# tsadja/ShaSTA

Measured on AMD Instinct MI355X. Metric: affinity frame-pairs/sec at N=M=500, F=256, higher is better.
Workload: dtype f32; 1 GPU; synthetic N=M=500, F=256 (num_point 4 x C 64), nf=7: affinity forward from HBM-resident NHWC BEV maps (SURVEY 8a rows 4-16); max_obj=500, num_feats=7, num_point=4, arithmetic=f16x2, parallelism=replica x1

## Files before the change

### shasta_amd/csrc/pair.hip

```cpp
#include "stages.hpp"
#include "pair_lane.hpp"

namespace shasta {

struct PackArgs {
    shasta_linear fs[4], fd[3], rc[3], aff0;
    float* out;
    int N, nf, F;
};

__device__ __forceinline__ void layer_src(const PackArgs& a, int l, const float*& W, const float*& b, int& ldw) {
    const PairDims d(a.F);
    switch (l) {
        case L_FS2: W = a.fs[1].weight; b = a.fs[1].bias; ldw = d.H1; break;
        case L_FS3: W = a.fs[2].weight; b = a.fs[2].bias; ldw = d.H2; break;
        case L_FS4: W = a.fs[3].weight; b = a.fs[3].bias; ldw = d.H3; break;
        case L_RC2: W = a.rc[1].weight; b = a.rc[1].bias; ldw = d.R1; break;
        case L_RC3: W = a.rc[2].weight; b = a.rc[2].bias; ldw = d.R2; break;
        case L_FD2: W = a.fd[1].weight; b = a.fd[1].bias; ldw = 32; break;
        default:    W = a.fd[2].weight; b = a.fd[2].bias; ldw = 8; break;
    }
}

__global__ void pack_pair_weights_kernel(PackArgs a) {
// ... 289 lines not shown
#pragma unroll
        for (int i = 0; i < TPI; ++i) dma_up(t + 2 * TPI + i, (t - t_beg + 2 * TPI + i) % RING);
        const int tt = t + th;
        unsigned upo = (unsigned)(unsigned long long)(my_up + ((t - t_beg + th) % RING) * UP_SLOT);
        asm volatile("" : "+v"(upo));
        const lfloat* up = (const lfloat*)(unsigned long long)upo;
        float hp[16];
        {
            const f32x4 h0 = *reinterpret_cast<const lf32x4*>(up + ET), h1 = *reinterpret_cast<const lf32x4*>(up + ET + 4),
                        h2 = *reinterpret_cast<const lf32x4*>(up + ET + 8), h3 = *reinterpret_cast<const lf32x4*>(up + ET + 12);
#pragma unroll
            for (int k = 0; k < 4; ++k) {
                hp[k] = h0[k];
                hp[4 + k] = h1[k];
                hp[8 + k] = h2[k];
                hp[12 + k] = h3[k];
            }
        }
        const lfloat *arow, *abias;
        a4l.per_track(arow, abias);

        auto layer12 = [&](auto tag, int seg, f32x4* acc) {
            using AL = decltype(tag);
            a4_init<AL>(abias, acc);
#pragma unroll
            for (int kg = 0; kg < AL::KG; ++kg) {
                const f32x4 u = *reinterpret_cast<const f32x4*>(ucrow + seg + 4 * kg);
                const f32x4 upv = *reinterpret_cast<const lf32x4*>(up + seg + 4 * kg);
                f32x4 a4[AL::NOB];
#pragma unroll
                for (int ob = 0; ob < AL::NOB; ++ob) a4[ob] = *reinterpret_cast<const lf32x4*>(arow + AL::OFF + (ob * AL::KG + kg) * 16);
#pragma unroll
                for (int kk = 0; kk < 4; ++kk) {
                    if (4 * kg + kk < AL::KIN) {
                        const float h = relu_nan(upv[kk] + u[kk]);
#pragma unroll
                        for (int ob = 0; ob < AL::NOB; ++ob) acc[ob] = MFMA4(a4[ob][kk], h, acc[ob]);
                    }
                }
            }
        };
        f32x4 a_rc2[A4<F, L_RC2>::NOB], a_rc3[A4<F, L_RC3>::NOB];
        f32x4 a_fs2[A4<F, L_FS2>::NOB], a_fs3[A4<F, L_FS3>::NOB], a_fs4[A4<F, L_FS4>::NOB];
        f32x4 a_fd2[A4<F, L_FD2>::NOB], a_fd3[A4<F, L_FD3>::NOB];
        layer12(A4<F, L_RC2>{}, H1, a_rc2);
        layer12(A4<F, L_FS2>{}, 0, a_fs2);
        layer12(A4<F, L_FD2>{}, H1 + R1, a_fd2);
        a4_layer<A4<F, L_RC3>, A4_RELU_NAN>(arow, abias, a_rc2, a_rc3);
        a4_layer<A4<F, L_FS3>, A4_RELU_NAN>(arow, abias, a_fs2, a_fs3);
        a4_layer<A4<F, L_FD3>, A4_RELU_NAN>(arow, abias, a_fd2, a_fd3);
        a4_layer<A4<F, L_FS4>, A4_RELU_NAN>(arow, abias, a_fs3, a_fs4);

        const float dist = hand_dist(hp, hd, dnm, rdn);
        const float res = pair_combine(a_rc3[0], a_fd3[0][0], dist, a_fs4[0][0]);
        if (d < D && tt < t_end) residual[((size_t)b * T + tt) * ld + d] = res;
    }
}

int pair_residual(const shasta_weights* w, const float* packed, int B, const float* feat, const float* prev_feat,
                  const float* det_tab, const float* prev_tab, float* residual, int ld, void* ws, size_t ws_bytes,
                  hipStream_t st, hipEvent_t ev0, hipEvent_t ev1) {
    const int N = w->max_obj, F = w->feat_dim, nf = w->num_feats, T = N + 2, D = N + 2;
    const PairDims d(F);
    const PackedLayout P(N, nf, F);
    const PairWs L(B, N, F);
    if (ws_bytes < L.total) {
        set_error_msg("pair_residual: workspace too small");
        return SHASTA_E_WORKSPACE;
    }
    if (B == 0) return SHASTA_OK;
    char* base = static_cast<char*>(ws);
    float* UP = reinterpret_cast<float*>(base + L.up);
    float* UC = reinterpret_cast<float*>(base + L.uc);
    float* hand_prev = reinterpret_cast<float*>(base + L.hand_prev);
// ... 112 lines not shown
```

### shasta_amd/csrc/pair_f16.hip

```cpp
#include "stages.hpp"
#include "pair_lane.hpp"
#include "pieces.hpp"

namespace shasta {


constexpr int P16_FRAG_DW = 2 * 4 * 64 * 4;

__global__ __launch_bounds__(256) void pair_f16_pack_kernel(PairF16PackArgs a) {
    __shared__ float red[3][4];
    __shared__ int ex[3];
    const int tid = threadIdx.x;
    const float* W[3] = {a.w_fs2, a.w_rc2, a.w_fd2};
    const int cnt[3] = {16 * 32, 16 * 64, 8 * 32};
    pair2_range_exponents(W, cnt, a.out, P16_FRAG_DW, red, ex);
    const int lane = tid & 63, frag = tid >> 6;
    const int i = lane & 15, kb = lane >> 4;
    const int mlp = frag == 0 ? 0 : frag == 3 ? 2 : 1;
    const int rows = mlp == 2 ? 8 : 16, kin = mlp == 1 ? 64 : 32, ks = frag == 2 ? 1 : 0;
    float v[8];
#pragma unroll
    for (int j = 0; j < 8; ++j) v[j] = i < rows ? __builtin_ldexpf(W[mlp][i * kin + 32 * ks + 8 * kb + j], ex[mlp]) : 0.0f;
    store_weight_pieces(v, a.out, 4, frag, lane);
}

int pair_f16_pack(const shasta_weights* w, float* out, hipStream_t st) {
    hipLaunchKernelGGL(pair_f16_pack_kernel, dim3(1), dim3(256), 0, st, pair_f16_pack_args(w, out));
    return check_launch("pair_f16_pack");
}

constexpr int PF_TS = 44;
constexpr int GR_ROW = 136;

template <int WPB, bool GRID>
struct PairF16Lds {
    static constexpr int US = PairDims(256).ET + 4;
    static constexpr int uc = 0;
    static constexpr int ucl = uc + 64 * (GR_ROW / 2);
    static constexpr int a4 = uc + (GRID ? 2 * 64 * (GR_ROW / 2) : 64 * US);
    static constexpr int up = a4 + pad4(a4_total(256));
    static constexpr int tr = up + WPB * 3 * UP_SLOT;
    static constexpr int upp = tr + WPB * 64 * PF_TS;
    static constexpr size_t bytes = (size_t)(upp + (GRID ? WPB * 128 : 0)) * sizeof(float);
};
static_assert(PairF16Lds<8, false>::bytes == 156912 && PairF16Lds<8, true>::bytes == 162032, "the sizes the launcher spelt out before");


template <int WPB, bool GRID>
__global__ __launch_bounds__(64 * WPB) void pair_f16_kernel(const float* __restrict__ packed, const uint32_t* __restrict__ p16,
                                                       const float* __restrict__ UP, const float* __restrict__ UC,
                                                       const float* __restrict__ hand_prev, const float* __restrict__ hand_det,
                                                       const float* __restrict__ denom, float* __restrict__ residual, int T,
                                                       int D, int ld, int nf, int TWG, int TA, int TB) {
    constexpr int F = 256;
    constexpr PairDims dm(F);
    constexpr int ET = dm.ET;
    static_assert(dm.H1 == 32 && dm.R1 == 64 && ET == 128 && dm.H2 == 16 && dm.R2 == 16, "pair_f16_kernel is laid out for F = 256");
    using Lds = PairF16Lds<WPB, GRID>;
    constexpr int US = Lds::US;
    extern __shared__ __attribute__((aligned(16))) float s_dynh[];
    float* s_uc = s_dynh + Lds::uc;
    float* s_a4 = s_dynh + Lds::a4;
    float* s_up = s_dynh + Lds::up;
    float* s_tr = s_dynh + Lds::tr;
    uint32_t* s_uch = reinterpret_cast<uint32_t*>(s_dynh + Lds::uc);
    uint32_t* s_ucl = reinterpret_cast<uint32_t*>(s_dynh + Lds::ucl);
    uint32_t* s_upp = reinterpret_cast<uint32_t*>(s_dynh + Lds::upp);
    const int tid = threadIdx.x, lane = tid & 63;
    const int wid = __builtin_amdgcn_readfirstlane(tid >> 6);
    int lbx, by, b;
    xcd_logical_block(lbx, by, b);
    const int d0 = lbx * 64;
    const int d = d0 + lane, dcl = min(d, D - 1);
    {
        if constexpr (!GRID) {
            const f32x4* src = reinterpret_cast<const f32x4*>(UC);
#pragma unroll 4
            for (int e = tid; e < 64 * (ET / 4); e += 64 * WPB) {
                const int r = e / (ET / 4), c = e - r * (ET / 4);
                const int cp = (((c >> 1) & 1) << 4) | (((c >> 2) & 1) << 3) | ((c >> 3) << 1) | (c & 1);
                *reinterpret_cast<f32x4*>(&s_uc[r * US + 4 * cp]) = src[((size_t)b * D + min(d0 + r, D - 1)) * (ET / 4) + c];
            }
        }
        a4_stage<F, 64 * WPB>(packed, s_a4, tid);
    }
    float hd[12];
    float mc = load_hand_det(hand_det + ((size_t)b * D + dcl) * 16, hd);
// ... 48 lines not shown
            _Float16 hh[4], ll[4];
#pragma unroll
            for (int q = 0; q < 4; ++q) {
                const float sv = __builtin_ldexpf(v[q], ex), hi = rintf(sv);
                hh[q] = (_Float16)hi;
                ll[q] = (_Float16)(rintf((sv - hi) * 2048.0f) * (1.0f / 2048.0f));
            }
            typedef uint32_t pu2 __attribute__((ext_vector_type(2)));
            typedef _Float16 ph2t __attribute__((ext_vector_type(2)));
            *reinterpret_cast<pu2*>(s_uch + r * (GR_ROW / 2) + 2 * c) =
                pu2{__builtin_bit_cast(uint32_t, ph2t{hh[0], hh[1]}), __builtin_bit_cast(uint32_t, ph2t{hh[2], hh[3]})};
            *reinterpret_cast<pu2*>(s_ucl + r * (GR_ROW / 2) + 2 * c) =
                pu2{__builtin_bit_cast(uint32_t, ph2t{ll[0], ll[1]}), __builtin_bit_cast(uint32_t, ph2t{ll[2], ll[3]})};
        }
    }
    u32x4 wh[4], wl[4];
#pragma unroll
    for (int f = 0; f < 4; ++f) {
        wh[f] = reinterpret_cast<const u32x4*>(p16)[(0 * 4 + f) * 64 + lane];
        wl[f] = reinterpret_cast<const u32x4*>(p16)[(1 * 4 + f) * 64 + lane];
    }
    const int ew_fs = reinterpret_cast<const int*>(p16)[P16_FRAG_DW + 0], ew_rc = reinterpret_cast<const int*>(p16)[P16_FRAG_DW + 1],
              ew_fd = reinterpret_cast<const int*>(p16)[P16_FRAG_DW + 2];
    __syncthreads();
    const A4Lane a4l(s_a4, lane);
    const f32x4 zero4 = {0, 0, 0, 0};
    const int p = lane & 15, kb = lane >> 4;
    float* my_tr = s_tr + wid * (64 * PF_TS);

    const int t_beg = by * TWG + (wid < 4 ? wid * TA : 4 * TA + (wid - 4) * TB);
    const int t_end = min(min(T, (by + 1) * TWG), t_beg + (wid < 4 ? TA : TB));
    float* my_up = s_up + wid * (3 * UP_SLOT);
    const bool hp_lane = lane >= ET / 4 && lane < ET / 4 + 4;
    const int up_lane = 4 * min(lane, ET / 4 - 1), hp_off = 4 * (lane - ET / 4);
    auto dma_up = [&](int row, int slot) {
        const size_t r = (size_t)b * T + min(row, T - 1);
        const float* src = hp_lane ? hand_prev + r * 16 + hp_off : UP + r * ET + up_lane;
        __builtin_amdgcn_global_load_lds((const __attribute__((address_space(1))) void*)src,
                                         (__attribute__((address_space(3))) void*)(my_up + slot * UP_SLOT), 16, 0, 0);
    };
    if (t_beg < t_end) {
        dma_up(t_beg, 0);
        dma_up(t_beg + 1, 1);
    }
    for (int t = t_beg; t < t_end; ++t) {
        asm volatile("s_waitcnt vmcnt(0)" ::: "memory");
        dma_up(t + 2, (t - t_beg + 2) % 3);
        unsigned upo = (unsigned)(unsigned long long)(my_up + ((t - t_beg) % 3) * UP_SLOT);
// ... 124 lines not shown
        {
            f32x4 ua[8], ub[8];
            u32x4 xha[4], xla[4], xhb[4], xlb[4];
            f32x4 fsA, rcA, fdA, fsB, rcB, fdB;
            load_uc(0, ua);
            load_uc(1, ub);
            cut(ua, xha, xla);
            load_uc(2, ua);
            cut(ub, xhb, xlb);
            mma(xha, xla, fsA, rcA, fdA);
            store(0, fsA, rcA, fdA);
            load_uc(3, ub);
            cut(ua, xha, xla);
            mma(xhb, xlb, fsB, rcB, fdB);
            store(1, fsB, rcB, fdB);
            cut(ub, xhb, xlb);
            mma(xha, xla, fsA, rcA, fdA);
            store(2, fsA, rcA, fdA);
            mma(xhb, xlb, fsB, rcB, fdB);
            store(3, fsB, rcB, fdB);
        }
        const lfloat *arow, *abias;
        a4l.per_track(arow, abias);
        const float i_rc = __builtin_ldexpf(1.0f, -((GRID ? ge[1] : e1) + ew_rc)), i_fs = __builtin_ldexpf(1.0f, -((GRID ? ge[0] : e1) + ew_fs)),
                    i_fd = __builtin_ldexpf(1.0f, -((GRID ? ge[2] : e1) + ew_fd));
        f32x4 a_rc2[4], a_fs2[4], a_fd2[2];
        {
            const float* mine = my_tr + lane * PF_TS;
            const float* b_rc = s_a4 + A4<F, L_RC2>::OFF + A4<F, L_RC2>::BIAS;
            const float* b_fs = s_a4 + A4<F, L_FS2>::OFF + A4<F, L_FS2>::BIAS;
            const float* b_fd = s_a4 + A4<F, L_FD2>::OFF + A4<F, L_FD2>::BIAS;
#pragma unroll
            for (int g = 0; g < 4; ++g) {
                a_rc2[g] = a4_descale_relu(*reinterpret_cast<const f32x4*>(mine + 4 * g), i_rc, *reinterpret_cast<const f32x4*>(b_rc + 4 * g));
                a_fs2[g] = a4_descale_relu(*reinterpret_cast<const f32x4*>(mine + 16 + 4 * g), i_fs, *reinterpret_cast<const f32x4*>(b_fs + 4 * g));
            }
#pragma unroll
            for (int g = 0; g < 2; ++g)
                a_fd2[g] = a4_descale_relu(*reinterpret_cast<const f32x4*>(mine + 32 + 4 * g), i_fd, *reinterpret_cast<const f32x4*>(b_fd + 4 * g));
        }
        asm volatile("" : "+v"(a_rc2[0]), "+v"(a_rc2[1]), "+v"(a_rc2[2]), "+v"(a_rc2[3]), "+v"(a_fs2[0]), "+v"(a_fs2[1]), "+v"(a_fs2[2]),
                     "+v"(a_fs2[3]), "+v"(a_fd2[0]), "+v"(a_fd2[1]));
        f32x4 a_rc3[A4<F, L_RC3>::NOB], a_fs3[A4<F, L_FS3>::NOB], a_fs4[A4<F, L_FS4>::NOB], a_fd3[A4<F, L_FD3>::NOB];
        {
            using RC = A4<F, L_RC3>;
            using FS = A4<F, L_FS3>;
            using FD = A4<F, L_FD3>;
            static_assert(RC::NOB == 1 && FS::NOB == 2 && FD::NOB == 1 && RC::KG == 4 && FS::KG == 4 && FD::KG == 2, "F = 256");
            a4_init<RC>(abias, a_rc3);
            a4_init<FS>(abias, a_fs3);
            a4_init<FD>(abias, a_fd3);
#pragma unroll
            for (int kg = 0; kg < 4; ++kg) {
                const f32x4 w_rc = *reinterpret_cast<const lf32x4*>(arow + RC::OFF + kg * 16);
                const f32x4 w_f0 = *reinterpret_cast<const lf32x4*>(arow + FS::OFF + kg * 16);
                const f32x4 w_f1 = *reinterpret_cast<const lf32x4*>(arow + FS::OFF + (FS::KG + kg) * 16);
                f32x4 w_fd = zero4;
                if (kg < 2) w_fd = *reinterpret_cast<const lf32x4*>(arow + FD::OFF + kg * 16);
#pragma unroll
                for (int kk = 0; kk < 4; ++kk) {
                    a_rc3[0] = MFMA4(w_rc[kk], a_rc2[kg][kk], a_rc3[0]);
                    a_fs3[0] = MFMA4(w_f0[kk], a_fs2[kg][kk], a_fs3[0]);
                    a_fs3[1] = MFMA4(w_f1[kk], a_fs2[kg][kk], a_fs3[1]);
                    if (kg < 2) a_fd3[0] = MFMA4(w_fd[kk], a_fd2[kg][kk], a_fd3[0]);
                }
            }
        }
        a4_layer<A4<F, L_FS4>, A4_RELU_FMAX>(arow, abias, a_fs3, a_fs4);

        const float dist = hand_dist(hp, hd, dnm, rdn);
        const float res = pair_combine(a_rc3[0], a_fd3[0][0], dist, a_fs4[0][0]);
        if (d < D) residual[((size_t)b * T + t) * ld + d] = finite_bound ? res : __builtin_nanf("");
    }
}

int launch_pair_f16(const float* packed, const float* p16, const float* UP, const float* UC, const float* hand_prev,
                    const float* hand_det, const float* denom, float* residual, int B, int T, int D, int ld, int nf, bool grid,
                    hipStream_t st) {
    constexpr int wpb = 8;
    int ny = 1;
    while ((long)B * cdiv(D, 64) * ny < 512 && cdiv(T, wpb * ny * 2) >= 2) ny *= 2;
    const int twg = cdiv(cdiv(T, ny), wpb) * wpb;
    int ta = twg / wpb, tb = ta;
    if (wpb == 8) {
        const int per_simd = twg / 4;
        ta = (per_simd * 1000 + (1000 + 615) / 2) / (1000 + 615);
        tb = per_simd - ta;
    }
    const size_t lds = grid ? PairF16Lds<wpb, true>::bytes : PairF16Lds<wpb, false>::bytes;
    dim3 grd(cdiv(D, 64), cdiv(T, twg), B);
    if (grid) {
        (void)hipFuncSetAttribute((const void*)pair_f16_kernel<wpb, true>, hipFuncAttributeMaxDynamicSharedMemorySize, (int)lds);
        hipLaunchKernelGGL((pair_f16_kernel<wpb, true>), grd, dim3(64 * wpb), lds, st, packed, reinterpret_cast<const uint32_t*>(p16), UP, UC,
                           hand_prev, hand_det, denom, residual, T, D, ld, nf, twg, ta, tb);
    } else {
// ... 9 lines not shown
```

### shasta_amd/csrc/pair_f16w.hip

```cpp
#include "stages.hpp"
#include "pair_lane.hpp"
#include "pieces.hpp"

namespace shasta {

template <int F>
struct PW {
    static constexpr PairDims dm{F};
    static constexpr int ET = dm.ET, H1 = dm.H1, R1 = dm.R1, H2 = dm.H2, R2 = dm.R2, NKS = ET / 16;
    static_assert(ET % 16 == 0 && H2 % 4 == 0 && H2 + 8 <= 32 && R2 <= 32, "wide pair tiles: 16-wide k steps, two 32-row output blocks");
    static constexpr bool has1(int ks) { return 16 * ks < H1 || 16 * ks + 16 > H1 + R1; }
    static constexpr bool has2(int ks) { return 16 * ks + 16 > H1 && 16 * ks < H1 + R1; }
    static constexpr int frag1(int ks) {
        int f = 0;
        for (int i = 0; i < ks; ++i) f += (has1(i) ? 1 : 0) + (has2(i) ? 1 : 0);
        return f;
    }
    static constexpr int frag2(int ks) { return frag1(ks) + (has1(ks) ? 1 : 0); }
    static constexpr int NFRAG = frag1(NKS);
    static constexpr int FRAG_DW = 2 * NFRAG * 64 * 4;
};
constexpr int P16W_MAX_DW = 2 * 16 * 64 * 4 + 4;
static_assert(PW<320>::FRAG_DW + 4 <= P16W_MAX_DW && PW<256>::FRAG_DW + 4 <= P16W_MAX_DW, "PackedLayout::p16w");

__device__ __forceinline__ f32x2 w_mul2(f32x2 a, f32x2 c) {
    f32x2 r;
    asm("v_pk_mul_f32 %0, %1, %2" : "=v"(r) : "v"(a), "v"(c));
    return r;
}

struct PairF16WPackArgs : PairF16PackArgs {};

template <int F>
__global__ __launch_bounds__(256) void pair_f16w_pack_kernel(PairF16WPackArgs a) {
    using W = PW<F>;
    __shared__ float red[3][4];
    __shared__ int ex[3];
    const int tid = threadIdx.x;
    const float* Wm[3] = {a.w_fs2, a.w_rc2, a.w_fd2};
    const int cnt[3] = {W::H2 * W::H1, W::R2 * W::R1, 8 * 32};
    pair2_range_exponents(Wm, cnt, a.out, W::FRAG_DW, red, ex);
    const int lane = tid & 63, m = lane & 31, kb = lane >> 5;
    for (int item = tid >> 6; item < 2 * W::NKS; item += 4) {
        const int ks = item >> 1, blk = item & 1;
        if (!(blk == 0 ? W::has1(ks) : W::has2(ks))) continue;
        const int frag = blk == 0 ? W::frag1(ks) : W::frag2(ks);
        float v[8];
#pragma unroll
        for (int j = 0; j < 8; ++j) {
            const int c = 16 * ks + 8 * kb + j;
            float x = 0.0f;
            if (blk == 0) {
                if (m < W::H2 && c < W::H1) x = __builtin_ldexpf(a.w_fs2[m * W::H1 + c], ex[0]);
                else if (m >= W::H2 && m < W::H2 + 8 && c >= W::H1 + W::R1) x = __builtin_ldexpf(a.w_fd2[(m - W::H2) * 32 + (c - W::H1 - W::R1)], ex[2]);
            } else if (m < W::R2 && c >= W::H1 && c < W::H1 + W::R1) {
                x = __builtin_ldexpf(a.w_rc2[m * W::R1 + (c - W::H1)], ex[1]);
            }
            v[j] = x;
        }
        store_weight_pieces(v, a.out, W::NFRAG, frag, lane);
    }
}

bool pair_f16w_serves(int F) { return F == 320; }

int pair_f16w_pack(const shasta_weights* w, float* out, hipStream_t st) {
    hipLaunchKernelGGL(pair_f16w_pack_kernel<320>, dim3(1), dim3(256), 0, st, PairF16WPackArgs{pair_f16_pack_args(w, out)});
    return check_launch("pair_f16w_pack");
}

constexpr int PWK_WPB = 4;

template <int F>
struct PairF16wLds {
    static constexpr int a4 = 0;
    static constexpr int up = a4 + pad4(a4_total(F));
    static constexpr int w = up + PWK_WPB * 6 * UP_SLOT;
    static constexpr size_t bytes = (size_t)(w + PW<F>::FRAG_DW) * sizeof(float);
};
static_assert(PairF16wLds<320>::bytes == 56928, "the size the launcher spelt out before");

template <int F>
__global__ __launch_bounds__(64 * PWK_WPB) __attribute__((amdgpu_waves_per_eu(2, 2))) void pair_f16w_kernel(const float* __restrict__ packed, const uint32_t* __restrict__ p16,
                                                               const float* __restrict__ UP, const float* __restrict__ UC,
                                                               const float* __restrict__ hand_prev, const float* __restrict__ hand_det,
                                                               const float* __restrict__ denom, float* __restrict__ residual, int T,
                                                               int D, int ld, int TWG) {
    using W = PW<F>;
    constexpr int ET = W::ET, NKS = W::NKS, NFRAG = W::NFRAG;
    using Lds = PairF16wLds<F>;
    extern __shared__ __attribute__((aligned(16))) float s_dynw[];
    float* s_a4 = s_dynw + Lds::a4;
    float* s_up = s_dynw + Lds::up;
    u32x4* s_w = reinterpret_cast<u32x4*>(s_dynw + Lds::w);
    const int tid = threadIdx.x, lane = tid & 63;
    const int wid = __builtin_amdgcn_readfirstlane(tid >> 6);
    int lbx, by, b;
    xcd_logical_block(lbx, by, b);
    const int d0 = lbx * 32;
    const int n = lane & 31, kb = lane >> 5;
    const int d = d0 + n, dcl = min(d, D - 1);
    a4_stage<F, 64 * PWK_WPB>(packed, s_a4, tid);
    f32x4 uc[NKS][2];
    {
        const f32x4* src = reinterpret_cast<const f32x4*>(UC + ((size_t)b * D + dcl) * ET);
#pragma unroll
        for (int ks = 0; ks < NKS; ++ks) {
            uc[ks][0] = src[4 * ks + 2 * kb];
            uc[ks][1] = src[4 * ks + 2 * kb + 1];
        }
    }
    float hd[12];
    float mc = load_hand_det(hand_det + ((size_t)b * D + dcl) * 16, hd);
#pragma unroll
    for (int off = 16; off > 0; off >>= 1) mc = absmax_keep_nan(mc, __shfl_xor(mc, off, 64));
    const float dnm = denom[(size_t)b * D + dcl], rdn = 1.0f / dnm;
    for (int e = tid; e < 2 * NFRAG * 64; e += 64 * PWK_WPB) s_w[e] = reinterpret_cast<const u32x4*>(p16)[e];
    const u32x4* my_w = s_w + lane;
    const int ew_fs = reinterpret_cast<const int*>(p16)[W::FRAG_DW + 0], ew_rc = reinterpret_cast<const int*>(p16)[W::FRAG_DW + 1],
              ew_fd = reinterpret_cast<const int*>(p16)[W::FRAG_DW + 2];
    __syncthreads();
    const A4Lane a4l(s_a4, lane);
    const f32x4 zero4 = {0, 0, 0, 0};
    const f32x16 zero16 = {0, 0, 0, 0, 0, 0, 0, 0, 0, 0, 0, 0, 0, 0, 0, 0};

    const int tw = TWG / PWK_WPB;
    const int t_beg = by * TWG + wid * tw;
    const int t_end = min(min(T, (by + 1) * TWG), t_beg + tw);
    float* my_up = s_up + wid * (6 * UP_SLOT);
    const bool hp_lane = lane >= ET / 4 && lane < ET / 4 + 4;
    const int up_lane = 4 * min(lane, ET / 4 - 1), hp_off = 4 * (lane - ET / 4);
    auto dma_up = [&](int row, int slot) __attribute__((always_inline)) {
        const size_t r = (size_t)b * T + min(row, T - 1);
        const float* src = hp_lane ? hand_prev + r * 16 + hp_off : UP + r * ET + up_lane;
        __builtin_amdgcn_global_load_lds((const __attribute__((address_space(1))) void*)src,
                                         (__attribute__((address_space(3))) void*)(my_up + slot * UP_SLOT), 16, 0, 0);
    };
    if (t_beg < t_end) {
        dma_up(t_beg, 0);
        dma_up(t_beg + 1, 1);
        dma_up(t_beg + 2, 2);
        dma_up(t_beg + 3, 3);
    }
// ... 95 lines not shown
                    q2[2 * g][r] = __uint_as_float(s2[0]);
                    q2[2 * g + 1][r] = __uint_as_float(s2[1]);
                }
            }
        const int my_t = t + kb;
        const lfloat* upL = upA + kb * UP_SLOT;
        float hp[16];
        {
            const f32x4 h0 = *reinterpret_cast<const lf32x4*>(upL + ET), h1 = *reinterpret_cast<const lf32x4*>(upL + ET + 4),
                        h2 = *reinterpret_cast<const lf32x4*>(upL + ET + 8), h3 = *reinterpret_cast<const lf32x4*>(upL + ET + 12);
#pragma unroll
            for (int k = 0; k < 4; ++k) {
                hp[k] = h0[k];
                hp[4 + k] = h1[k];
                hp[8 + k] = h2[k];
                hp[12 + k] = h3[k];
            }
        }
        const float bound = kb ? boundB : boundA;
        const bool finite_bound = bound < INFINITY;
        const int e1 = kb ? e1B : e1A;
        const lfloat *arow, *abias;
        a4l.per_track(arow, abias);
        const float i_rc = __builtin_ldexpf(1.0f, -(e1 + ew_rc)), i_fs = __builtin_ldexpf(1.0f, -(e1 + ew_fs)), i_fd = __builtin_ldexpf(1.0f, -(e1 + ew_fd));
        constexpr int NQ_FS = W::H2 / 4, NQ_RC = (W::R2 + 3) / 4;
        f32x4 a_fs2[NQ_FS], a_rc2[NQ_RC], a_fd2[2];
        {
            const float* b_rc = s_a4 + A4<F, L_RC2>::OFF + A4<F, L_RC2>::BIAS;
            const float* b_fs = s_a4 + A4<F, L_FS2>::OFF + A4<F, L_FS2>::BIAS;
            const float* b_fd = s_a4 + A4<F, L_FD2>::OFF + A4<F, L_FD2>::BIAS;
#pragma unroll
            for (int g = 0; g < NQ_FS; ++g) a_fs2[g] = a4_descale_relu(q1[g], i_fs, *reinterpret_cast<const f32x4*>(b_fs + 4 * g));
#pragma unroll
            for (int g = 0; g < 2; ++g) a_fd2[g] = a4_descale_relu(q1[NQ_FS + g], i_fd, *reinterpret_cast<const f32x4*>(b_fd + 4 * g));
#pragma unroll
            for (int g = 0; g < NQ_RC; ++g) a_rc2[g] = a4_descale_relu(q2[g], i_rc, *reinterpret_cast<const f32x4*>(b_rc + 4 * g));
        }
        f32x4 a_rc3[A4<F, L_RC3>::NOB], a_fs3[A4<F, L_FS3>::NOB], a_fs4[A4<F, L_FS4>::NOB], a_fd3[A4<F, L_FD3>::NOB];
        {
            using FS = A4<F, L_FS3>;
            using RC = A4<F, L_RC3>;
            using FD = A4<F, L_FD3>;
            static_assert(RC::NOB == 1 && FD::NOB == 1 && FD::KG == 2, "third layers: res_coeff -> 3, fuse_det -> 1");
            a4_init<FS>(abias, a_fs3);
            a4_init<RC>(abias, a_rc3);
            a4_init<FD>(abias, a_fd3);
            constexpr int KGM = FS::KG > RC::KG ? FS::KG : RC::KG;
#pragma unroll
            for (int kg = 0; kg < KGM; ++kg) {
                f32x4 w_fs[FS::NOB], w_rc = zero4, w_fd = zero4;
#pragma unroll
                for (int ob = 0; ob < FS::NOB; ++ob)
                    if (kg < FS::KG) w_fs[ob] = *reinterpret_cast<const lf32x4*>(arow + FS::OFF + (ob * FS::KG + kg) * 16);
                if (kg < RC::KG) w_rc = *reinterpret_cast<const lf32x4*>(arow + RC::OFF + kg * 16);
                if (kg < FD::KG) w_fd = *reinterpret_cast<const lf32x4*>(arow + FD::OFF + kg * 16);
#pragma unroll
                for (int kk = 0; kk < 4; ++kk) {
                    if (kg < FS::KG && 4 * kg + kk < FS::KIN)
#pragma unroll
                        for (int ob = 0; ob < FS::NOB; ++ob) a_fs3[ob] = MFMA4(w_fs[ob][kk], a_fs2[kg][kk], a_fs3[ob]);
                    if (kg < RC::KG && 4 * kg + kk < RC::KIN) a_rc3[0] = MFMA4(w_rc[kk], a_rc2[kg][kk], a_rc3[0]);
                    if (kg < FD::KG) a_fd3[0] = MFMA4(w_fd[kk], a_fd2[kg][kk], a_fd3[0]);
                }
            }
        }
        a4_layer<A4<F, L_FS4>, A4_RELU_FMAX>(arow, abias, a_fs3, a_fs4);
        const float dist = hand_dist(hp, hd, dnm, rdn);
        const float res = pair_combine(a_rc3[0], a_fd3[0][0], dist, a_fs4[0][0]);
        if (d < D && my_t < t_end) residual[((size_t)b * T + my_t) * ld + d] = finite_bound ? res : __builtin_nanf("");
    }
}

int launch_pair_f16w(const float* packed, const float* p16, const float* UP, const float* UC, const float* hand_prev,
                     const float* hand_det, const float* denom, float* residual, int B, int T, int D, int ld, int F, hipStream_t st) {
    if (F != 320) {
        set_error_msg("launch_pair_f16w: feat_dim must be 320");
        return SHASTA_E_ARG;
    }
    constexpr int unit = 2 * PWK_WPB;
    int ny = 1;
    while ((long)B * cdiv(D, 32) * ny < 512 && cdiv(T, unit * ny * 2) >= 2) ny *= 2;
    while ((long)B * cdiv(D, 32) * ny < 256 && cdiv(T, unit * ny * 2) >= 1) ny *= 2;
    const int twg = cdiv(cdiv(T, ny), unit) * unit;
    constexpr size_t lds = PairF16wLds<320>::bytes;
    dim3 grd(cdiv(D, 32), cdiv(T, twg), B);
    if (hipFuncSetAttribute((const void*)pair_f16w_kernel<320>, hipFuncAttributeMaxDynamicSharedMemorySize, (int)lds) != hipSuccess) {
        (void)hipGetLastError();
        set_error_msg("pair_f16w: the device does not grant the kernel's LDS per workgroup");
        return SHASTA_E_UNSUPPORTED;
    }
    hipLaunchKernelGGL((pair_f16w_kernel<320>), grd, dim3(64 * PWK_WPB), lds, st, packed, reinterpret_cast<const uint32_t*>(p16), UP, UC,
                       hand_prev, hand_det, denom, residual, T, D, ld, twg);
// ... 5 lines not shown
```

### shasta_amd/csrc/pair_lane.hpp

```cpp
#pragma once
#include "common.hpp"
#include "pair_layout.hpp"
#include "pieces.hpp"

namespace shasta {

typedef __attribute__((address_space(3))) float lfloat;
typedef __attribute__((address_space(3))) f32x4 lf32x4;

constexpr int UP_SLOT = 256;

#define MFMA4(a, b, c) __builtin_amdgcn_mfma_f32_4x4x1f32((a), (b), (c), 0, 0, 0)

template <int F, int L>
struct A4 {
    static constexpr LayerDesc D = layer_desc(F, L);
    static constexpr int NOB = a4_nob(F, L), KG = a4_kg(F, L), OFF = a4_offset(F, L), KIN = D.kin, BIAS = NOB * KG * 16;
};

template <int F, int NT>
__device__ __forceinline__ void a4_stage(const float* __restrict__ packed, float* s_a4, const int& tid) {
    const PackedLayout P(0, 0, F);
    const f32x4* asrc = reinterpret_cast<const f32x4*>(packed + P.a4);
#pragma unroll 2
    for (int e = tid; e < a4_total(F) / 4; e += NT) reinterpret_cast<f32x4*>(s_a4)[e] = asrc[e];
}

struct A4Lane {
    unsigned arow_base, abias_base;
    __device__ __forceinline__ A4Lane(const float* s_a4, int lane)
        : arow_base((unsigned)(unsigned long long)(s_a4 + (lane & 3) * 4)), abias_base((unsigned)(unsigned long long)(s_a4 + (lane & 3))) {}
    __device__ __forceinline__ void per_track(const lfloat*& arow, const lfloat*& abias) const {
        unsigned ao = arow_base, bo = abias_base;
        asm volatile("" : "+v"(ao), "+v"(bo));
        arow = (const lfloat*)(unsigned long long)ao;
        abias = (const lfloat*)(unsigned long long)bo;
    }
};

template <class AL>
__device__ __forceinline__ void a4_init(const lfloat* abias, f32x4* acc) {
    const f32x4 zero4 = {0, 0, 0, 0};
#pragma unroll
    for (int ob = 0; ob < AL::NOB; ++ob) acc[ob] = MFMA4(abias[AL::OFF + AL::BIAS + ob * 4], 1.0f, zero4);
}

enum A4Relu { A4_RELU_FMAX, A4_RELU_NAN };

template <class AL, A4Relu RELU>
__device__ __forceinline__ void a4_layer(const lfloat* arow, const lfloat* abias, const f32x4* in, f32x4* acc) {
    a4_init<AL>(abias, acc);
#pragma unroll
    for (int kg = 0; kg < AL::KG; ++kg) {
        f32x4 a4[AL::NOB];
#pragma unroll
        for (int ob = 0; ob < AL::NOB; ++ob) a4[ob] = *reinterpret_cast<const lf32x4*>(arow + AL::OFF + (ob * AL::KG + kg) * 16);
#pragma unroll
        for (int kk = 0; kk < 4; ++kk) {
            if (4 * kg + kk < AL::KIN) {
                const float h = RELU == A4_RELU_NAN ? relu_nan(in[kg][kk]) : fmaxf(in[kg][kk], 0.0f);
#pragma unroll
                for (int ob = 0; ob < AL::NOB; ++ob) acc[ob] = MFMA4(a4[ob][kk], h, acc[ob]);
            }
        }
    }
}

__device__ __forceinline__ f32x4 a4_descale_relu(const f32x4& v, float sc, const f32x4& bb) {
    const f32x2 s2 = {sc, sc};
    const f32x2 lo = __builtin_elementwise_fma(f32x2{v[0], v[1]}, s2, f32x2{bb[0], bb[1]});
    const f32x2 hi = __builtin_elementwise_fma(f32x2{v[2], v[3]}, s2, f32x2{bb[2], bb[3]});
    return f32x4{fmaxf(lo[0], 0.0f), fmaxf(lo[1], 0.0f), fmaxf(hi[0], 0.0f), fmaxf(hi[1], 0.0f)};
}

__device__ __forceinline__ float load_hand_det(const float* row, float (&hd)[12]) {
    const f32x4* h = reinterpret_cast<const f32x4*>(row);
    const f32x4 a = h[0], c = h[1], e = h[2], g = h[3];
    hd[0] = a[0]; hd[1] = a[1]; hd[2] = a[2]; hd[3] = a[3]; hd[4] = c[0]; hd[5] = c[1]; hd[6] = c[2];
    hd[7] = e[0]; hd[8] = e[1]; hd[9] = e[2]; hd[10] = e[3]; hd[11] = g[0];
    return g[1];
}

__device__ __forceinline__ float hand_dist(const float (&hp)[16], const float (&hd)[12], float dnm, float rdn) {
    typedef float hpf2 __attribute__((ext_vector_type(2)));
    hpf2 d01 = hpf2{hp[0], hp[1]} - hpf2{hd[0], hd[1]}, d23 = hpf2{hp[2], hp[3]} - hpf2{hd[2], hd[3]},
         d45 = hpf2{hp[4], hp[5]} - hpf2{hd[4], hd[5]};
    const float d6 = hp[6] - hd[6];
    d01 *= d01;
    d23 *= d23;
    d45 *= d45;
    const float d2 = (((((d01[0] + d01[1]) + d23[0]) + d23[1]) + d45[0]) + d45[1]) + d6 * d6;
    const float q = d2 * rdn;
    const float r = __builtin_fmaf(__builtin_fmaf(-q, dnm, d2), rdn, q);
    const float dim = (__builtin_fabsf(hp[8] - hd[7]) + __builtin_fabsf(hp[9] - hd[8])) + __builtin_fabsf(hp[10] - hd[9]);
    hpf2 cs = hpf2{hp[11], hp[12]} - hpf2{hd[10], hd[11]};
// ... 9 lines not shown
    const float* w_fs2;
    const float* w_rc2;
    const float* w_fd2;
    uint32_t* out;
};

inline PairF16PackArgs pair_f16_pack_args(const shasta_weights* w, float* out) {
    return {w->fuse_shape[1].weight, w->res_coeff[1].weight, w->fuse_det[1].weight, reinterpret_cast<uint32_t*>(out)};
}

__device__ __forceinline__ void store_weight_pieces(const float (&v)[8], uint32_t* out, int nfrag, int frag, int lane) {
    u32x4 hi, lo;
#pragma unroll
    for (int j = 0; j < 4; ++j) {
        const _Float16 h0 = (_Float16)v[2 * j], h1 = (_Float16)v[2 * j + 1];
        const f16x2 hh = {h0, h1};
        hi[j] = __builtin_bit_cast(uint32_t, hh);
        lo[j] = cvt_f16x2(v[2 * j] - (float)h0, v[2 * j + 1] - (float)h1);
    }
    reinterpret_cast<u32x4*>(out)[(0 * nfrag + frag) * 64 + lane] = hi;
    reinterpret_cast<u32x4*>(out)[(1 * nfrag + frag) * 64 + lane] = lo;
}

__device__ __forceinline__ void pair2_range_exponents(const float* const (&W)[3], const int (&cnt)[3], uint32_t* out, int at,
                                                      float (&red)[3][4], int (&ex)[3]) {
    const int tid = threadIdx.x;
    for (int m = 0; m < 3; ++m) {
        float mx = 0.0f;
        for (int i = tid; i < cnt[m]; i += 256) mx = fmaxf(mx, fabsf(W[m][i]));
#pragma unroll
        for (int off = 32; off > 0; off >>= 1) mx = fmaxf(mx, __shfl_xor(mx, off, 64));
        if ((tid & 63) == 0) red[m][tid >> 6] = mx;
    }
    __syncthreads();
    if (tid < 3) {
        const float mx = fmaxf(fmaxf(red[tid][0], red[tid][1]), fmaxf(red[tid][2], red[tid][3]));
        ex[tid] = range_exponent_bits(__float_as_uint(mx));
        reinterpret_cast<int*>(out)[at + tid] = ex[tid];
    }
    if (tid == 3) out[at + 3] = 0;
    __syncthreads();
}

}
```

Measured before the change: 65970 frame-pairs/s.

## Prescale layer-2 activations to clamp f16 range and fold relu clamp

Adds a per-workgroup setup that bounds the layer-2 pre-activation magnitude from the track hand rows, the bias, and a packed row-L1 weight bound. It then rescales the descale exponent and the biases by a power of two, so layer-2 outputs fit a clamped range via fma2_relu01. Later layers are scaled back up at the end, and NaN is emitted when the bound overflows. This appears aimed at a cheaper fused fma+clamp replacing fma+fmax. It adds a reduction prologue, a small LDS bias table, and extra multiplies.

```diff
diff --git a/shasta_amd/csrc/pair.hip b/shasta_amd/csrc/pair.hip
--- a/shasta_amd/csrc/pair.hip
+++ b/shasta_amd/csrc/pair.hip
@@ -335,7 +335,7 @@
 
         auto layer12 = [&](auto tag, int seg, f32x4* acc) {
             using AL = decltype(tag);
-            a4_init<AL>(abias, acc);
+            a4_init<AL>(abias, acc, 1.0f);
 #pragma unroll
             for (int kg = 0; kg < AL::KG; ++kg) {
                 const f32x4 u = *reinterpret_cast<const f32x4*>(ucrow + seg + 4 * kg);
@@ -359,10 +359,10 @@
         layer12(A4<F, L_RC2>{}, H1, a_rc2);
         layer12(A4<F, L_FS2>{}, 0, a_fs2);
         layer12(A4<F, L_FD2>{}, H1 + R1, a_fd2);
-        a4_layer<A4<F, L_RC3>, A4_RELU_NAN>(arow, abias, a_rc2, a_rc3);
-        a4_layer<A4<F, L_FS3>, A4_RELU_NAN>(arow, abias, a_fs2, a_fs3);
-        a4_layer<A4<F, L_FD3>, A4_RELU_NAN>(arow, abias, a_fd2, a_fd3);
-        a4_layer<A4<F, L_FS4>, A4_RELU_NAN>(arow, abias, a_fs3, a_fs4);
+        a4_layer<A4<F, L_RC3>, A4_RELU_NAN>(arow, abias, a_rc2, a_rc3, 1.0f);
+        a4_layer<A4<F, L_FS3>, A4_RELU_NAN>(arow, abias, a_fs2, a_fs3, 1.0f);
+        a4_layer<A4<F, L_FD3>, A4_RELU_NAN>(arow, abias, a_fd2, a_fd3, 1.0f);
+        a4_layer<A4<F, L_FS4>, A4_RELU_NAN>(arow, abias, a_fs3, a_fs4, 1.0f);
 
         const float dist = hand_dist(hp, hd, dnm, rdn);
         const float res = pair_combine(a_rc3[0], a_fd3[0][0], dist, a_fs4[0][0]);
diff --git a/shasta_amd/csrc/pair_f16.hip b/shasta_amd/csrc/pair_f16.hip
--- a/shasta_amd/csrc/pair_f16.hip
+++ b/shasta_amd/csrc/pair_f16.hip
@@ -12,8 +12,8 @@
     __shared__ int ex[3];
     const int tid = threadIdx.x;
     const float* W[3] = {a.w_fs2, a.w_rc2, a.w_fd2};
-    const int cnt[3] = {16 * 32, 16 * 64, 8 * 32};
-    pair2_range_exponents(W, cnt, a.out, P16_FRAG_DW, red, ex);
+    const int cnt[3] = {16 * 32, 16 * 64, 8 * 32}, kin3[3] = {32, 64, 32};
+    pair2_range_exponents(W, cnt, kin3, a.out, P16_FRAG_DW, red, ex);
     const int lane = tid & 63, frag = tid >> 6;
     const int i = lane & 15, kb = lane >> 4;
     const int mlp = frag == 0 ? 0 : frag == 3 ? 2 : 1;
@@ -41,9 +41,11 @@
     static constexpr int up = a4 + pad4(a4_total(256));
     static constexpr int tr = up + WPB * 3 * UP_SLOT;
     static constexpr int upp = tr + WPB * 64 * PF_TS;
-    static constexpr size_t bytes = (size_t)(upp + (GRID ? WPB * 128 : 0)) * sizeof(float);
+    static constexpr int b2 = upp + (GRID ? WPB * 128 : 0);
+    static constexpr size_t bytes = (size_t)(b2 + L2Bias<256>::N) * sizeof(float);
 };
-static_assert(PairF16Lds<8, false>::bytes == 156912 && PairF16Lds<8, true>::bytes == 162032, "the sizes the launcher spelt out before");
+static_assert(PairF16Lds<8, false>::bytes == 156912 + 160 && PairF16Lds<8, true>::bytes == 162032 + 160 && PairF16Lds<8, true>::bytes <= 160 * 1024,
+              "the sizes the launcher spelt out before + the scaled bias table; one workgroup per CU");
 
 
 template <int WPB, bool GRID>
@@ -63,6 +65,7 @@
     float* s_a4 = s_dynh + Lds::a4;
     float* s_up = s_dynh + Lds::up;
     float* s_tr = s_dynh + Lds::tr;
+    float* s_b2 = s_dynh + Lds::b2;
     uint32_t* s_uch = reinterpret_cast<uint32_t*>(s_dynh + Lds::uc);
     uint32_t* s_ucl = reinterpret_cast<uint32_t*>(s_dynh + Lds::ucl);
     uint32_t* s_upp = reinterpret_cast<uint32_t*>(s_dynh + Lds::upp);
@@ -157,8 +160,15 @@
     }
     const int ew_fs = reinterpret_cast<const int*>(p16)[P16_FRAG_DW + 0], ew_rc = reinterpret_cast<const int*>(p16)[P16_FRAG_DW + 1],
               ew_fd = reinterpret_cast<const int*>(p16)[P16_FRAG_DW + 2];
+    const int tw0 = by * TWG;
+    const L2Clamp l2 = l2_clamp_setup<F>(packed, hand_prev + ((size_t)b * T + tw0) * 16, min(T, tw0 + TWG) - tw0, mc,
+                                         __uint_as_float(p16[P16_FRAG_DW + 3]), s_b2, tid);
+    const int em_fs = ew_fs + l2.m, em_rc = ew_rc + l2.m, em_fd = ew_fd + l2.m;
     __syncthreads();
     const A4Lane a4l(s_a4, lane);
+    unsigned b2o = (unsigned)(unsigned long long)s_b2;
+    asm volatile("" : "+v"(b2o));
+    const lfloat* l_b2 = (const lfloat*)(unsigned long long)b2o;
     const f32x4 zero4 = {0, 0, 0, 0};
     const int p = lane & 15, kb = lane >> 4;
     float* my_tr = s_tr + wid * (64 * PF_TS);
@@ -329,24 +339,27 @@
         }
         const lfloat *arow, *abias;
         a4l.per_track(arow, abias);
-        const float i_rc = __builtin_ldexpf(1.0f, -((GRID ? ge[1] : e1) + ew_rc)), i_fs = __builtin_ldexpf(1.0f, -((GRID ? ge[0] : e1) + ew_fs)),
-                    i_fd = __builtin_ldexpf(1.0f, -((GRID ? ge[2] : e1) + ew_fd));
+        const float i_rc = __builtin_ldexpf(1.0f, -((GRID ? ge[1] : e1) + em_rc)), i_fs = __builtin_ldexpf(1.0f, -((GRID ? ge[0] : e1) + em_fs)),
+                    i_fd = __builtin_ldexpf(1.0f, -((GRID ? ge[2] : e1) + em_fd));
         f32x4 a_rc2[4], a_fs2[4], a_fd2[2];
         {
             const float* mine = my_tr + lane * PF_TS;
-            const float* b_rc = s_a4 + A4<F, L_RC2>::OFF + A4<F, L_RC2>::BIAS;
-            const float* b_fs = s_a4 + A4<F, L_FS2>::OFF + A4<F, L_FS2>::BIAS;
-            const float* b_fd = s_a4 + A4<F, L_FD2>::OFF + A4<F, L_FD2>::BIAS;
+            const lfloat* b_rc = l_b2 + L2Bias<F>::RC;
+            const lfloat* b_fs = l_b2 + L2Bias<F>::FS;
+            const lfloat* b_fd = l_b2 + L2Bias<F>::FD;
 #pragma unroll
             for (int g = 0; g < 4; ++g) {
-                a_rc2[g] = a4_descale_relu(*reinterpret_cast<const f32x4*>(mine + 4 * g), i_rc, *reinterpret_cast<const f32x4*>(b_rc + 4 * g));
-                a_fs2[g] = a4_descale_relu(*reinterpret_cast<const f32x4*>(mine + 16 + 4 * g), i_fs, *reinterpret_cast<const f32x4*>(b_fs + 4 * g));
-            }
-#pragma unroll
-            for (int g = 0; g < 2; ++g)
-                a_fd2[g] = a4_descale_relu(*reinterpret_cast<const f32x4*>(mine + 32 + 4 * g), i_fd, *reinterpret_cast<const f32x4*>(b_fd + 4 * g));
-        }
-        asm volatile("" : "+v"(a_rc2[0]), "+v"(a_rc2[1]), "+v"(a_rc2[2]), "+v"(a_rc2[3]), "+v"(a_fs2[0]), "+v"(a_fs2[1]), "+v"(a_fs2[2]),
+                const f32x4 bq_rc = *reinterpret_cast<const lf32x4*>(b_rc + 4 * g), bq_fs = *reinterpret_cast<const lf32x4*>(b_fs + 4 * g);
+                a_rc2[g] = a4_descale_clamp(*reinterpret_cast<const f32x4*>(mine + 4 * g), i_rc, bq_rc);
+                a_fs2[g] = a4_descale_clamp(*reinterpret_cast<const f32x4*>(mine + 16 + 4 * g), i_fs, bq_fs);
+            }
+#pragma unroll
+            for (int g = 0; g < 2; ++g) {
+                const f32x4 bq = *reinterpret_cast<const lf32x4*>(b_fd + 4 * g);
+                a_fd2[g] = a4_descale_clamp(*reinterpret_cast<const f32x4*>(mine + 32 + 4 * g), i_fd, bq);
+            }
+        }
+        asm volatile("s_nop 1" : "+v"(a_rc2[0]), "+v"(a_rc2[1]), "+v"(a_rc2[2]), "+v"(a_rc2[3]), "+v"(a_fs2[0]), "+v"(a_fs2[1]), "+v"(a_fs2[2]),
                      "+v"(a_fs2[3]), "+v"(a_fd2[0]), "+v"(a_fd2[1]));
         f32x4 a_rc3[A4<F, L_RC3>::NOB], a_fs3[A4<F, L_FS3>::NOB], a_fs4[A4<F, L_FS4>::NOB], a_fd3[A4<F, L_FD3>::NOB];
         {
@@ -354,9 +367,9 @@
             using FS = A4<F, L_FS3>;
             using FD = A4<F, L_FD3>;
             static_assert(RC::NOB == 1 && FS::NOB == 2 && FD::NOB == 1 && RC::KG == 4 && FS::KG == 4 && FD::KG == 2, "F = 256");
-            a4_init<RC>(abias, a_rc3);
-            a4_init<FS>(abias, a_fs3);
-            a4_init<FD>(abias, a_fd3);
+            a4_init<RC>(abias, a_rc3, l2.dn);
+            a4_init<FS>(abias, a_fs3, l2.dn);
+            a4_init<FD>(abias, a_fd3, l2.dn);
 #pragma unroll
             for (int kg = 0; kg < 4; ++kg) {
                 const f32x4 w_rc = *reinterpret_cast<const lf32x4*>(arow + RC::OFF + kg * 16);
@@ -373,11 +386,12 @@
                 }
             }
         }
-        a4_layer<A4<F, L_FS4>, A4_RELU_FMAX>(arow, abias, a_fs3, a_fs4);
+        a4_layer<A4<F, L_FS4>, A4_RELU_FMAX>(arow, abias, a_fs3, a_fs4, l2.dn);
 
         const float dist = hand_dist(hp, hd, dnm, rdn);
-        const float res = pair_combine(a_rc3[0], a_fd3[0][0], dist, a_fs4[0][0]);
-        if (d < D) residual[((size_t)b * T + t) * ld + d] = finite_bound ? res : __builtin_nanf("");
+        const f32x4 rc = {a_rc3[0][0] * l2.up, a_rc3[0][1] * l2.up, a_rc3[0][2] * l2.up, 0.0f};
+        const float res = pair_combine(rc, a_fd3[0][0] * l2.up, dist, a_fs4[0][0] * l2.up);
+        if (d < D) residual[((size_t)b * T + t) * ld + d] = finite_bound && l2.ok ? res : __builtin_nanf("");
     }
 }
 
diff --git a/shasta_amd/csrc/pair_f16w.hip b/shasta_amd/csrc/pair_f16w.hip
--- a/shasta_amd/csrc/pair_f16w.hip
+++ b/shasta_amd/csrc/pair_f16w.hip
@@ -38,8 +38,8 @@
     __shared__ int ex[3];
     const int tid = threadIdx.x;
     const float* Wm[3] = {a.w_fs2, a.w_rc2, a.w_fd2};
-    const int cnt[3] = {W::H2 * W::H1, W::R2 * W::R1, 8 * 32};
-    pair2_range_exponents(Wm, cnt, a.out, W::FRAG_DW, red, ex);
+    const int cnt[3] = {W::H2 * W::H1, W::R2 * W::R1, 8 * 32}, kin3[3] = {W::H1, W::R1, 32};
+    pair2_range_exponents(Wm, cnt, kin3, a.out, W::FRAG_DW, red, ex);
     const int lane = tid & 63, m = lane & 31, kb = lane >> 5;
     for (int item = tid >> 6; item < 2 * W::NKS; item += 4) {
         const int ks = item >> 1, blk = item & 1;
@@ -76,9 +76,11 @@
     static constexpr int a4 = 0;
     static constexpr int up = a4 + pad4(a4_total(F));
     static constexpr int w = up + PWK_WPB * 6 * UP_SLOT;
-    static constexpr size_t bytes = (size_t)(w + PW<F>::FRAG_DW) * sizeof(float);
+    static constexpr int b2 = w + PW<F>::FRAG_DW;
+    static constexpr size_t bytes = (size_t)(b2 + L2Bias<F>::N) * sizeof(float);
 };
-static_assert(PairF16wLds<320>::bytes == 56928, "the size the launcher spelt out before");
+static_assert(PairF16wLds<320>::bytes == 56928 + 192 && 2 * PairF16wLds<320>::bytes <= 160 * 1024,
+              "the size the launcher spelt out before + the scaled bias table; two workgroups per CU");
 
 template <int F>
 __global__ __launch_bounds__(64 * PWK_WPB) __attribute__((amdgpu_waves_per_eu(2, 2))) void pair_f16w_kernel(const float* __restrict__ packed, const uint32_t* __restrict__ p16,
@@ -93,6 +95,7 @@
     float* s_a4 = s_dynw + Lds::a4;
     float* s_up = s_dynw + Lds::up;
     u32x4* s_w = reinterpret_cast<u32x4*>(s_dynw + Lds::w);
+    float* s_b2 = s_dynw + Lds::b2;
     const int tid = threadIdx.x, lane = tid & 63;
     const int wid = __builtin_amdgcn_readfirstlane(tid >> 6);
     int lbx, by, b;
@@ -119,6 +122,10 @@
     const u32x4* my_w = s_w + lane;
     const int ew_fs = reinterpret_cast<const int*>(p16)[W::FRAG_DW + 0], ew_rc = reinterpret_cast<const int*>(p16)[W::FRAG_DW + 1],
               ew_fd = reinterpret_cast<const int*>(p16)[W::FRAG_DW + 2];
+    const int tw0 = by * TWG;
+    const L2Clamp l2 = l2_clamp_setup<F>(packed, hand_prev + ((size_t)b * T + tw0) * 16, min(T, tw0 + TWG) - tw0, mc,
+                                         __uint_as_float(p16[W::FRAG_DW + 3]), s_b2, tid);
+    const int em_fs = ew_fs + l2.m, em_rc = ew_rc + l2.m, em_fd = ew_fd + l2.m;
     __syncthreads();
     const A4Lane a4l(s_a4, lane);
     const f32x4 zero4 = {0, 0, 0, 0};
@@ -260,29 +267,32 @@
         const int e1 = kb ? e1B : e1A;
         const lfloat *arow, *abias;
         a4l.per_track(arow, abias);
-        const float i_rc = __builtin_ldexpf(1.0f, -(e1 + ew_rc)), i_fs = __builtin_ldexpf(1.0f, -(e1 + ew_fs)), i_fd = __builtin_ldexpf(1.0f, -(e1 + ew_fd));
+        const float i_rc = __builtin_ldexpf(1.0f, -(e1 + em_rc)), i_fs = __builtin_ldexpf(1.0f, -(e1 + em_fs)), i_fd = __builtin_ldexpf(1.0f, -(e1 + em_fd));
         constexpr int NQ_FS = W::H2 / 4, NQ_RC = (W::R2 + 3) / 4;
         f32x4 a_fs2[NQ_FS], a_rc2[NQ_RC], a_fd2[2];
         {
-            const float* b_rc = s_a4 + A4<F, L_RC2>::OFF + A4<F, L_RC2>::BIAS;
-            const float* b_fs = s_a4 + A4<F, L_FS2>::OFF + A4<F, L_FS2>::BIAS;
-            const float* b_fd = s_a4 + A4<F, L_FD2>::OFF + A4<F, L_FD2>::BIAS;
-#pragma unroll
-            for (int g = 0; g < NQ_FS; ++g) a_fs2[g] = a4_descale_relu(q1[g], i_fs, *reinterpret_cast<const f32x4*>(b_fs + 4 * g));
-#pragma unroll
-            for (int g = 0; g < 2; ++g) a_fd2[g] = a4_descale_relu(q1[NQ_FS + g], i_fd, *reinterpret_cast<const f32x4*>(b_fd + 4 * g));
-#pragma unroll
-            for (int g = 0; g < NQ_RC; ++g) a_rc2[g] = a4_descale_relu(q2[g], i_rc, *reinterpret_cast<const f32x4*>(b_rc + 4 * g));
-        }
+            const float* b_rc = s_b2 + L2Bias<F>::RC;
+            const float* b_fs = s_b2 + L2Bias<F>::FS;
+            const float* b_fd = s_b2 + L2Bias<F>::FD;
+#pragma unroll
+            for (int g = 0; g < NQ_FS; ++g) a_fs2[g] = a4_descale_clamp(q1[g], i_fs, *reinterpret_cast<const f32x4*>(b_fs + 4 * g));
+#pragma unroll
+            for (int g = 0; g < 2; ++g) a_fd2[g] = a4_descale_clamp(q1[NQ_FS + g], i_fd, *reinterpret_cast<const f32x4*>(b_fd + 4 * g));
+#pragma unroll
+            for (int g = 0; g < NQ_RC; ++g) a_rc2[g] = a4_descale_clamp(q2[g], i_rc, *reinterpret_cast<const f32x4*>(b_rc + 4 * g));
+        }
+        static_assert(NQ_FS == 5 && NQ_RC == 5, "the pin below names every quad");
+        asm volatile("s_nop 1" : "+v"(a_fs2[0]), "+v"(a_fs2[1]), "+v"(a_fs2[2]), "+v"(a_fs2[3]), "+v"(a_fs2[4]), "+v"(a_rc2[0]), "+v"(a_rc2[1]),
+                     "+v"(a_rc2[2]), "+v"(a_rc2[3]), "+v"(a_rc2[4]), "+v"(a_fd2[0]), "+v"(a_fd2[1]));
         f32x4 a_rc3[A4<F, L_RC3>::NOB], a_fs3[A4<F, L_FS3>::NOB], a_fs4[A4<F, L_FS4>::NOB], a_fd3[A4<F, L_FD3>::NOB];
         {
             using FS = A4<F, L_FS3>;
             using RC = A4<F, L_RC3>;
             using FD = A4<F, L_FD3>;
             static_assert(RC::NOB == 1 && FD::NOB == 1 && FD::KG == 2, "third layers: res_coeff -> 3, fuse_det -> 1");
-            a4_init<FS>(abias, a_fs3);
-            a4_init<RC>(abias, a_rc3);
-            a4_init<FD>(abias, a_fd3);
+            a4_init<FS>(abias, a_fs3, l2.dn);
+            a4_init<RC>(abias, a_rc3, l2.dn);
+            a4_init<FD>(abias, a_fd3, l2.dn);
             constexpr int KGM = FS::KG > RC::KG ? FS::KG : RC::KG;
 #pragma unroll
             for (int kg = 0; kg < KGM; ++kg) {
@@ -302,10 +312,11 @@
                 }
             }
         }
-        a4_layer<A4<F, L_FS4>, A4_RELU_FMAX>(arow, abias, a_fs3, a_fs4);
+        a4_layer<A4<F, L_FS4>, A4_RELU_FMAX>(arow, abias, a_fs3, a_fs4, l2.dn);
         const float dist = hand_dist(hp, hd, dnm, rdn);
-        const float res = pair_combine(a_rc3[0], a_fd3[0][0], dist, a_fs4[0][0]);
-        if (d < D && my_t < t_end) residual[((size_t)b * T + my_t) * ld + d] = finite_bound ? res : __builtin_nanf("");
+        const f32x4 rc = {a_rc3[0][0] * l2.up, a_rc3[0][1] * l2.up, a_rc3[0][2] * l2.up, 0.0f};
+        const float res = pair_combine(rc, a_fd3[0][0] * l2.up, dist, a_fs4[0][0] * l2.up);
+        if (d < D && my_t < t_end) residual[((size_t)b * T + my_t) * ld + d] = finite_bound && l2.ok ? res : __builtin_nanf("");
     }
 }
 
diff --git a/shasta_amd/csrc/pair_lane.hpp b/shasta_amd/csrc/pair_lane.hpp
--- a/shasta_amd/csrc/pair_lane.hpp
+++ b/shasta_amd/csrc/pair_lane.hpp
@@ -39,17 +39,17 @@
 };
 
 template <class AL>
-__device__ __forceinline__ void a4_init(const lfloat* abias, f32x4* acc) {
+__device__ __forceinline__ void a4_init(const lfloat* abias, f32x4* acc, float sc) {
     const f32x4 zero4 = {0, 0, 0, 0};
 #pragma unroll
-    for (int ob = 0; ob < AL::NOB; ++ob) acc[ob] = MFMA4(abias[AL::OFF + AL::BIAS + ob * 4], 1.0f, zero4);
+    for (int ob = 0; ob < AL::NOB; ++ob) acc[ob] = MFMA4(abias[AL::OFF + AL::BIAS + ob * 4], sc, zero4);
 }
 
 enum A4Relu { A4_RELU_FMAX, A4_RELU_NAN };
 
 template <class AL, A4Relu RELU>
-__device__ __forceinline__ void a4_layer(const lfloat* arow, const lfloat* abias, const f32x4* in, f32x4* acc) {
-    a4_init<AL>(abias, acc);
+__device__ __forceinline__ void a4_layer(const lfloat* arow, const lfloat* abias, const f32x4* in, f32x4* acc, float sc) {
+    a4_init<AL>(abias, acc, sc);
 #pragma unroll
     for (int kg = 0; kg < AL::KG; ++kg) {
         f32x4 a4[AL::NOB];
@@ -66,11 +66,58 @@
     }
 }
 
-__device__ __forceinline__ f32x4 a4_descale_relu(const f32x4& v, float sc, const f32x4& bb) {
+__device__ __forceinline__ f32x4 a4_descale_clamp(const f32x4& v, float sc, const f32x4& bb) {
     const f32x2 s2 = {sc, sc};
-    const f32x2 lo = __builtin_elementwise_fma(f32x2{v[0], v[1]}, s2, f32x2{bb[0], bb[1]});
-    const f32x2 hi = __builtin_elementwise_fma(f32x2{v[2], v[3]}, s2, f32x2{bb[2], bb[3]});
-    return f32x4{fmaxf(lo[0], 0.0f), fmaxf(lo[1], 0.0f), fmaxf(hi[0], 0.0f), fmaxf(hi[1], 0.0f)};
+    const f32x2 lo = fma2_relu01(f32x2{v[0], v[1]}, s2, f32x2{bb[0], bb[1]});
+    const f32x2 hi = fma2_relu01(f32x2{v[2], v[3]}, s2, f32x2{bb[2], bb[3]});
+    return f32x4{lo[0], lo[1], hi[0], hi[1]};
+}
+
+template <int F>
+struct L2Bias {
+    static constexpr int NRC = A4<F, L_RC2>::NOB * 4, NFS = A4<F, L_FS2>::NOB * 4, NFD = A4<F, L_FD2>::NOB * 4;
+    static constexpr int RC = 0, FS = NRC, FD = NRC + NFS, N = NRC + NFS + NFD;
+    static_assert(N <= 64, "one lane per bias");
+    static __device__ __forceinline__ int src(int j) {
+        return j < FS   ? A4<F, L_RC2>::OFF + A4<F, L_RC2>::BIAS + j
+               : j < FD ? A4<F, L_FS2>::OFF + A4<F, L_FS2>::BIAS + (j - FS)
+                        : A4<F, L_FD2>::OFF + A4<F, L_FD2>::BIAS + (j - FD);
+    }
+};
+
+struct L2Clamp {
+    int m;
+    float dn, up;
+    bool ok;
+};
+
+template <int F>
+__device__ __forceinline__ L2Clamp l2_clamp_setup(const float* __restrict__ packed, const float* __restrict__ rows, int ntr, float mc,
+                                                  float R, float* s_b2, int tid) {
+    using LB = L2Bias<F>;
+    const int lane = tid & 63;
+    const PackedLayout P(0, 0, F);
+    const float bias = lane < LB::N ? packed[P.a4 + LB::src(lane)] : 0.0f;
+    float h = 0.0f, bm = fabsf(bias);
+    for (int t = lane; t < ntr; t += 64) {
+        const float v = rows[(size_t)t * 16 + 13] + mc;
+        h = v < INFINITY ? fmaxf(h, v) : h;
+    }
+#pragma unroll
+    for (int off = 32; off > 0; off >>= 1) {
+        h = fmaxf(h, __shfl_xor(h, off, 64));
+        bm = fmaxf(bm, __shfl_xor(bm, off, 64));
+    }
+    const float s = h * R + bm;
+    L2Clamp c;
+    c.ok = s < 0x1p119f;
+    int ex = -64;
+    if (c.ok && s > 0.0f) (void)frexpf(s, &ex);
+    c.m = max(-32, min(120, ex + 1));
+    c.dn = __builtin_ldexpf(1.0f, -c.m);
+    c.up = __builtin_ldexpf(1.0f, c.m);
+    if (tid < LB::N) s_b2[tid] = bias * c.dn;
+    return c;
 }
 
 __device__ __forceinline__ float load_hand_det(const float* row, float (&hd)[12]) {
@@ -126,8 +173,9 @@
     reinterpret_cast<u32x4*>(out)[(1 * nfrag + frag) * 64 + lane] = lo;
 }
 
-__device__ __forceinline__ void pair2_range_exponents(const float* const (&W)[3], const int (&cnt)[3], uint32_t* out, int at,
-                                                      float (&red)[3][4], int (&ex)[3]) {
+__device__ __forceinline__ void pair2_range_exponents(const float* const (&W)[3], const int (&cnt)[3], const int (&kin)[3], uint32_t* out,
+                                                      int at, float (&red)[3][4], int (&ex)[3]) {
+    __shared__ float rowl1[4];
     const int tid = threadIdx.x;
     for (int m = 0; m < 3; ++m) {
         float mx = 0.0f;
@@ -136,13 +184,26 @@
         for (int off = 32; off > 0; off >>= 1) mx = fmaxf(mx, __shfl_xor(mx, off, 64));
         if ((tid & 63) == 0) red[m][tid >> 6] = mx;
     }
+    float l1 = 0.0f;
+    for (int m = 0; m < 3; ++m)
+        if (tid < cnt[m] / kin[m]) {
+            float sum = 0.0f;
+            for (int k = 0; k < kin[m]; ++k) sum += fabsf(W[m][tid * kin[m] + k]);
+            l1 = absmax_keep_nan(l1, sum);
+        }
+#pragma unroll
+    for (int off = 32; off > 0; off >>= 1) l1 = absmax_keep_nan(l1, __shfl_xor(l1, off, 64));
+    if ((tid & 63) == 0) rowl1[tid >> 6] = l1;
     __syncthreads();
     if (tid < 3) {
         const float mx = fmaxf(fmaxf(red[tid][0], red[tid][1]), fmaxf(red[tid][2], red[tid][3]));
         ex[tid] = range_exponent_bits(__float_as_uint(mx));
         reinterpret_cast<int*>(out)[at + tid] = ex[tid];
     }
-    if (tid == 3) out[at + 3] = 0;
+    if (tid == 3) {
+        const float r = absmax_keep_nan(absmax_keep_nan(rowl1[0], rowl1[1]), absmax_keep_nan(rowl1[2], rowl1[3]));
+        out[at + 3] = __float_as_uint(r * (1.0f + 0x1p-12f));
+    }
     __syncthreads();
 }
 
```

Result: no change. 66370 frame-pairs/s (median of 6 runs) (+0.6%).
